# mirams/PyHillFit

Measured on NVIDIA B200. Metric: chain-iterations/sec (all chains, device-timed), higher is better.
Workload: dtype f64

## Files before the change

### pyhillfit_b200/csrc/phf_math.cuh

```cuda
#pragma once
#include <cstdint>
#include <cuda_runtime.h>
#include <math_constants.h>

#include "phf_fastmath.cuh"

#define PHF_DI __device__ __forceinline__
#if PHF_FM_TABLE_MODE == 1
#define PHF_STAGE_FASTMATH_TABLE(T)                                   \
    __shared__ __align__(16) double T##_smem[PHF_FM_TABLE_SIZE];      \
    phf::fm::stage_table(T##_smem);                                   \
    __syncthreads();                                                  \
    const double *const T = T##_smem
#elif PHF_FM_LUT
#define PHF_STAGE_FASTMATH_TABLE(T)                                                                     \
    __shared__ __align__(16) double T##_lut[PHF_FM_LUT_SIZE];                                           \
    for (int i_ = threadIdx.x; i_ < PHF_FM_LUT_SIZE; i_ += blockDim.x) T##_lut[i_] = phf::fm::kFmLut[i_]; \
    __syncthreads();                                                                                    \
    const double *const T = T##_lut
#else
#define PHF_STAGE_FASTMATH_TABLE(T) const double *const T = phf::fm::kFmTable
#endif

namespace phf {

constexpr double kSigmaLower = 1e-3;
constexpr double kPic50ExpRate = 0.2;
constexpr double kPic50ExpLower = -3.0;
constexpr double kHillLower = 0.0;
constexpr double kHillUpper = 10.0;
constexpr double kSigmaShapeM1 = 4.0;
constexpr double kSigmaScale = (6.0 - 1e-3) / (5.0 - 1.0);
constexpr double kLn10Hi = 2.302585092994045901e+00;
constexpr double kLn10Lo = -2.170756223382249351e-16;
constexpr double kSqrtHalf = 7.071067811865475244e-01;
constexpr double kPivotFloor = 1e-12;

__device__ __forceinline__ double guarded_pivot(double s, double diag)
{
    const double fl = kPivotFloor * diag;
    return s > fl ? s : fl;
}

PHF_DI double adapt_gamma(const double *T, uint32_t t, uint32_t adapt_when)
{
    return t > adapt_when ? fm::exp_clamped(T, -0.6 * fm::log_pos(T, (double)(t - adapt_when) + 1.0)) : 0.0;
}

template <int G>
PHF_DI unsigned group_mask()
{
    return G == 32 ? 0xffffffffu : (((1u << (G & 31)) - 1u) << (threadIdx.x & 31u & ~(unsigned)(G - 1)));
}

template <int G>
PHF_DI double group_sum(double v, unsigned mask)
{
#pragma unroll
    for (int o = G / 2; o > 0; o >>= 1) v += __shfl_xor_sync(mask, v, o, G);
    return v;
}

struct Philox4 {
    uint32_t w[4];
};

#ifndef PHF_PHILOX_ROUNDS
#define PHF_PHILOX_ROUNDS 10
#endif
PHF_DI Philox4 philox4x32_10(uint32_t c0, uint32_t c1, uint32_t c2, uint32_t c3, uint32_t k0, uint32_t k1)
{
#pragma unroll
    for (int r = 0; r < PHF_PHILOX_ROUNDS; ++r) {
        const uint32_t hi0 = __umulhi(0xD2511F53u, c0), lo0 = 0xD2511F53u * c0;
        const uint32_t hi1 = __umulhi(0xCD9E8D57u, c2), lo1 = 0xCD9E8D57u * c2;
        c0 = hi1 ^ c1 ^ k0;
        c1 = lo1;
        c2 = hi0 ^ c3 ^ k1;
        c3 = lo0;
        k0 += 0x9E3779B9u;
        k1 += 0xBB67AE85u;
    }
    Philox4 o;
    o.w[0] = c0; o.w[1] = c1; o.w[2] = c2; o.w[3] = c3;
    return o;
}

PHF_DI Philox4 philox_call(uint64_t seed, uint64_t chain, uint32_t t, uint32_t j)
{
    return philox4x32_10(t, j, (uint32_t)chain, (uint32_t)(chain >> 32), (uint32_t)seed, (uint32_t)(seed >> 32));
}

PHF_DI double uniform53(uint32_t w0, uint32_t w1)
{
    const unsigned long long v = (((unsigned long long)w0 << 32) | w1) >> 11;
    return fma((double)v, 0x1p-53, 0x1p-54);
}

PHF_DI void box_muller(const double *T, uint32_t a, uint32_t b, double &z0, double &z1)
{
    const double u1 = fma((double)a, 0x1p-32, 0x1p-32);
    const double r = fm::sqrt_nonneg(-2.0 * fm::log_pos(T, u1));
    double s, c;
    fm::sincos_turn32(T, b, s, c);
    z0 = r * c;
    z1 = r * s;
}

PHF_DI double log_ndtr_nonpos(const double *T, double z) { return fm::log_ndtr_nonpos(T, z); }

PHF_DI double ndtr(double a)
{
    const double x = a * kSqrtHalf, z = fabs(x);
    double y;
    if (z < 1.0)
        y = 0.5 + 0.5 * erf(x);
    else {
        y = 0.5 * erfc(z);
        if (x > 0) y = 1.0 - y;
    }
    return y;
}

PHF_DI void ln_ic50(double pic50, double &hi, double &lo)
{
    const double a = 6.0 - pic50;
    hi = a * kLn10Hi;
    lo = fma(a, kLn10Lo, fma(a, kLn10Hi, -hi));
}

template <bool ZERO_POW = true>
PHF_DI double hill_ratio_pow(const double *T, double lnc_hi, double lnc_lo, double lic_hi, double lic_lo, double hill)
{
    const double L = (lnc_hi - lic_hi) + (lnc_lo - lic_lo);
    const double x = fm::exp_clamped(T, hill * L);
    return (ZERO_POW && hill == 0.0) ? 1.0 : x;
}

PHF_DI double hill_response(double x) { return fma(-100.0, fm::rcp(1.0 + x), 100.0); }

}
```

### pyhillfit_b200/csrc/phf_single.cu

```cuda
#include "phf_common.cuh"
#include "phf_single.cuh"

namespace phf {

template <int MODEL>
__global__ void __launch_bounds__(128) log_target_batch_kernel(int64_t n, const double *__restrict__ theta,
                                                               const int32_t *__restrict__ dataset_id,
                                                               const double *__restrict__ temperature,
                                                               const phf_dataset *__restrict__ datasets,
                                                               const phf_dose_group *__restrict__ groups,
                                                               double *__restrict__ log_target,
                                                               double *__restrict__ loglik_t1)
{
    constexpr int D = SingleDims<MODEL>::D;
    PHF_STAGE_FASTMATH_TABLE(T);
    const int64_t i = (int64_t)blockIdx.x * blockDim.x + threadIdx.x;
    if (i >= n) return;
    double th[D];
#pragma unroll
    for (int k = 0; k < D; ++k) th[k] = theta[i * D + k];
    const phf_dataset ds = datasets[dataset_id[i]];
    double lt, l1;
    single_log_target<MODEL>(T, th, groups + ds.group_begin, ds.n_groups, ds.pi_bit, ds.n_other_total, temperature[i],
                             lt, l1);
    log_target[i] = lt;
    if (loglik_t1) loglik_t1[i] = l1;
}

template <int MODEL>
__global__ void __launch_bounds__(128) am_single_init_kernel(int64_t n, const double *__restrict__ theta0,
                                                             const double *__restrict__ cov0,
                                                             const int32_t *__restrict__ dataset_id,
                                                             const double *__restrict__ temperature,
                                                             const phf_dataset *__restrict__ datasets,
                                                             const phf_dose_group *__restrict__ groups,
                                                             double *__restrict__ state)
{
    constexpr int D = SingleDims<MODEL>::D, NT = SingleDims<MODEL>::NT, NF = SingleDims<MODEL>::NF;
    PHF_STAGE_FASTMATH_TABLE(T);
    const int64_t i = (int64_t)blockIdx.x * blockDim.x + threadIdx.x;
    if (i >= n) return;
    double th[D];
#pragma unroll
    for (int k = 0; k < D; ++k) th[k] = theta0[i * D + k];
    const phf_dataset ds = datasets[dataset_id[i]];
    double lt, l1;
    single_log_target<MODEL>(T, th, groups + ds.group_begin, ds.n_groups, ds.pi_bit, ds.n_other_total, temperature[i],
                             lt, l1);
    double *s = state + i * NF;
#pragma unroll
    for (int k = 0; k < D; ++k) {
        s[k] = th[k];
        s[PHF_STATE_MEAN(D) + k] = th[k];
    }
    s[PHF_STATE_LOG_TARGET(D)] = lt;
    s[PHF_STATE_LOGLIK_T1(D)] = l1;
    {
        int q = 0;
#pragma unroll
        for (int r = 0; r < D; ++r)
#pragma unroll
            for (int c2 = 0; c2 <= r; ++c2, ++q) {
                const double v = cov0[i * NT + q];
                s[PHF_STATE_COV(D) + q] = (r == c2 && !(v > 0.0) && v == v) ? PHF_COV0_DIAG_FLOOR : v;
            }
    }
    s[PHF_STATE_LOGA(D)] = 0.0;
    s[PHF_STATE_LOGLIK_T1_SUM(D)] = 0.0;
    s[PHF_STATE_N_ACCEPTED(D)] = 0.0;
}

struct ChainConst {
    const phf_dose_group *grp;
    int ng;
    double pi_bit, n_other_total, temp;
    uint32_t thinning, adapt_when, burn_rows, row_base;
    int reset_mean;
    PrepView pv;
    double *out;
    size_t row_stride;
    bool active;
};

template <int MODEL, int G>
PHF_DI void am_step(const double *T, const ChainConst &cc, ChainRegs<MODEL> &s, const Draws<SingleDims<MODEL>::D> &dr,
                    double gam, uint32_t t, int gl, unsigned mask, uint32_t &until_save, uint32_t &row)
{
    constexpr int D = SingleDims<MODEL>::D;
    double star[D];
    propose<MODEL>(T, s.th, s.cov, s.loga, dr.z, star);

    double lt_star, l1_star;
    single_log_target_lanes<MODEL, G, true, true>(T, star, cc.grp, cc.ng, cc.pi_bit, cc.n_other_total, cc.temp, gl, mask,
                                                  lt_star, l1_star, cc.pv);
    const bool accepted = dr.log_u < lt_star - s.lt;
    if (accepted) {
#pragma unroll
        for (int k = 0; k < D; ++k) s.th[k] = star[k];
        s.lt = lt_star;
        s.l1 = l1_star;
        s.n_acc += 1.0;
    }

    if (cc.reset_mean && t == cc.adapt_when) {
#pragma unroll
        for (int k = 0; k < D; ++k) s.mean[k] = s.th[k];
    }
    adapt_update<D>(s.mean, s.cov, s.loga, s.th, gam, (accepted ? 1.0 : 0.0) - 0.25);

    if (--until_save == 0u) {
        until_save = cc.thinning;
        ++row;
        if (cc.out && cc.active && row >= cc.row_base) {
            double *o = cc.out + (size_t)(row - cc.row_base) * cc.row_stride;
#pragma unroll
            for (int k = 0; k <= D; ++k)
                if ((k & (G - 1)) == gl) o[k] = k < D ? s.th[k < D ? k : 0] : s.lt;
        }
        if (row >= cc.burn_rows) s.l1_sum += s.l1;
    }
}

constexpr int kOrderClasses = 8;
constexpr int kOrderMaxGrid = 4096;

__device__ __forceinline__ int ordered_block_index(int cta_chains, const int32_t *__restrict__ dataset_id,
                                                   const phf_dataset *__restrict__ datasets,
                                                   const phf_dose_group *__restrict__ groups)
{
    __shared__ unsigned char cls[kOrderMaxGrid];
    __shared__ int count[kOrderClasses], my_class, my_rank, chosen;
    const int tid = threadIdx.x, n_ctas = gridDim.x;
    if (tid < kOrderClasses) count[tid] = 0;
    __syncthreads();
    for (int b = tid; b < n_ctas; b += blockDim.x) {
        const phf_dataset ds = datasets[dataset_id[(int64_t)b * cta_chains]];
        int w = ds.n_groups > 4 ? ds.n_groups - 4 : 0;
        for (int g = 0; g < ds.n_groups && g < 16; ++g) {
            const phf_dose_group &Gd = groups[ds.group_begin + g];
            w += (Gd.n0 > 0.0 ? 1 : 0) + (Gd.n100 > 0.0 ? 1 : 0);
        }
        w = w < kOrderClasses ? w : kOrderClasses - 1;
        cls[b] = (unsigned char)w;
        atomicAdd(&count[w], 1);
    }
    __syncthreads();
    if (tid == 0) {
        int p = blockIdx.x, c = kOrderClasses - 1;
        for (; c > 0 && p >= count[c]; --c) p -= count[c];
        my_class = c;
        my_rank = p;
    }
    __syncthreads();
    if (tid < 32) {
        const int want = my_class, rank = my_rank;
        int seen = 0;
        for (int base = 0; base < n_ctas; base += 32) {
            const int b = base + tid;
            const unsigned m = __ballot_sync(0xffffffffu, b < n_ctas && cls[b] == want);
            const int here = __popc(m);
            if (seen + here > rank) {
                if (tid == 0) chosen = base + (int)__fns(m, 0, rank - seen + 1);
                break;
            }
            seen += here;
        }
    }
    __syncthreads();
    return chosen;
}

template <int MODEL, int G, int MINB>
__global__ void __launch_bounds__(128, MINB)
    am_single_kernel(phf_am_config cfg, int64_t n, double *__restrict__ state, const int32_t *__restrict__ dataset_id,
                     const double *__restrict__ temperature, const phf_dataset *__restrict__ datasets,
                     const phf_dose_group *__restrict__ groups, double *__restrict__ samples, int ordered)
{
    constexpr int D = SingleDims<MODEL>::D, NF = SingleDims<MODEL>::NF;
    extern __shared__ __align__(16) unsigned char smem_raw[];
    phf_dose_group *sgroups = reinterpret_cast<phf_dose_group *>(smem_raw);
    PHF_STAGE_FASTMATH_TABLE(T);

    const int cta_chains = blockDim.x / G;
    const int64_t first = (int64_t)(ordered ? ordered_block_index(cta_chains, dataset_id, datasets, groups)
                                            : (int)blockIdx.x) * cta_chains;
    const int64_t chain = first + threadIdx.x / G;
    const int gl = threadIdx.x & (G - 1);
    const bool active = chain < n;
    const int64_t c = active ? chain : n - 1;
    const unsigned lane = threadIdx.x & 31u;
    const unsigned mask = 0xffffffffu;

    const phf_dataset ds = datasets[dataset_id[c]];
    ChainConst cc;
    cc.grp = ds.n_groups > 0 ? groups + ds.group_begin : groups;
    if (cfg.stage_groups > 0) {
        const int64_t last = min(first + (int64_t)cta_chains, n) - 1;
        const phf_dataset d_lo = datasets[dataset_id[first]];
        const phf_dataset d_hi = datasets[dataset_id[last]];
        const int g_lo = d_lo.group_begin, g_hi = d_hi.group_begin + d_hi.n_groups;
        const bool fits = (g_hi - g_lo) <= cfg.stage_groups && g_hi > g_lo && ds.group_begin >= g_lo &&
                          ds.group_begin + ds.n_groups <= g_hi;
        const int all_fit = __syncthreads_and(fits ? 1 : 0);
        if (all_fit) {
            const double2 *src = reinterpret_cast<const double2 *>(groups + g_lo);
            double2 *dst = reinterpret_cast<double2 *>(sgroups);
            const int nvec = (g_hi - g_lo) * 4;
            for (int v = threadIdx.x; v < nvec; v += blockDim.x) dst[v] = __ldg(src + v);
            __syncthreads();
            cc.grp = sgroups + (ds.n_groups > 0 ? ds.group_begin - g_lo : 0);
        }
    }
    cc.ng = ds.n_groups;
    cc.pi_bit = ds.pi_bit;
    cc.n_other_total = ds.n_other_total;
    cc.temp = temperature[c];
    cc.thinning = cfg.thinning;
    cc.adapt_when = cfg.adapt_when;
    cc.burn_rows = cfg.burn_rows;
    cc.reset_mean = cfg.reset_mean_at_adapt;
    cc.active = active;
    const uint64_t chain_id = cfg.chain_id_base + (uint64_t)c;

    double *sp = state + c * NF;
    ChainRegs<MODEL> s;
    s.load(sp);

    uint32_t t = cfg.t0;
    uint32_t until_save = cfg.thinning - (t % cfg.thinning);
    uint32_t row = t / cfg.thinning;
    cc.row_base = first_row_written(cfg);
    const bool row_major = cfg.sample_layout == PHF_SAMPLES_ROW_MAJOR;
    cc.out = samples ? samples + (row_major ? (size_t)c : (size_t)c * cfg.rows_capacity) * (D + 1) : nullptr;
    cc.row_stride = row_major ? (size_t)n * (D + 1) : (size_t)(D + 1);

    double *const slots = reinterpret_cast<double *>(smem_raw + (size_t)cfg.stage_groups * sizeof(phf_dose_group));
    double *const gam_base = slots + (G > 1 ? (size_t)blockDim.x * (D + 1) : 0);
    double *const gam_slots = gam_base + (size_t)(threadIdx.x & ~31u);
    {
        constexpr int U = 4 / G;
        double2 *const prep = reinterpret_cast<double2 *>(gam_base + blockDim.x) + threadIdx.x;
        bool both = false;
#pragma unroll
        for (int u = 0; u < U; ++u)
            prepare_group<MODEL>(cc.grp, gl + u * G, cc.ng, prep + (size_t)(u * kPrepPairs) * blockDim.x, (int)blockDim.x, both);
        cc.pv = PrepView{prep, (int)blockDim.x, both};
    }

    double *const my_slot = slots + (size_t)threadIdx.x * (D + 1);
    const double *const chain_slots = slots + (size_t)(threadIdx.x & ~(unsigned)(G - 1)) * (D + 1);
    for (uint32_t it = 0; it < cfg.n_iters; ++it) {
        ++t;
        if ((it & 31u) == 0u) {
            const double gam_lane = adapt_gamma(T, t + lane, cfg.adapt_when);
            __syncwarp();
            gam_slots[lane] = gam_lane;
            __syncwarp();
        }
        const double gam = gam_slots[it & 31u];
        Draws<D> dr;
        if (G == 1) {
            dr = make_draws<D>(T, cfg.seed, chain_id, t);
        } else {
            const int slot = (int)(it & (uint32_t)(G - 1));
            if (slot == 0) {
                const Draws<D> mine = make_draws<D>(T, cfg.seed, chain_id, t + (uint32_t)gl);
                __syncwarp();
                my_slot[0] = mine.log_u;
#pragma unroll
                for (int k = 0; k < D; ++k) my_slot[1 + k] = mine.z[k];
                __syncwarp();
            }
            const double *src = chain_slots + slot * (D + 1);
            dr.log_u = src[0];
#pragma unroll
            for (int k = 0; k < D; ++k) dr.z[k] = src[1 + k];
        }
        am_step<MODEL, G>(T, cc, s, dr, gam, t, gl, mask, until_save, row);
    }

    if (active && gl == 0) s.store(sp);
}

template <int MODEL, int G, int MINB>
static int launch_am_single(const phf_am_config &cfg, int64_t n, int block, double *state, const int32_t *dataset_id,
                            const double *temperature, const phf_dataset *datasets, const phf_dose_group *groups,
                            double *samples, cudaStream_t s)
{
    constexpr int D = SingleDims<MODEL>::D;
    auto kern = am_single_kernel<MODEL, G, MINB>;
    const size_t smem = (size_t)cfg.stage_groups * sizeof(phf_dose_group) +
                        (G > 1 ? (size_t)block * (D + 1) * sizeof(double) : 0) + (size_t)block * sizeof(double) +
                        (size_t)block * (4 / G) * 64;
    if (int rc = allow_dynamic_smem(kern, smem)) return rc;
    const int cta_chains = block / G;
    const unsigned grid = (unsigned)((n + cta_chains - 1) / cta_chains);
    const int ordered = cfg.cta_order == 0 && grid > (unsigned)sm_count() && grid <= (unsigned)kOrderMaxGrid;
    kern<<<grid, block, smem, s>>>(cfg, n, state, dataset_id, temperature, datasets, groups, samples, ordered);
    count_launch();
    return check_launch("am_single_kernel");
}

int am_single_spec_launch(const phf_am_config &cfg, int lanes, int depth, int64_t n, int block, double *state,
                          const int32_t *dataset_id, const double *temperature, const phf_dataset *datasets,
                          const phf_dose_group *groups, double *samples, cudaStream_t s);

}

using namespace phf;

extern "C" int phf_log_target_batch(int model, int64_t n, const double *theta, const int32_t *dataset_id,
                                    const double *temperature, const phf_dataset *datasets,
                                    const phf_dose_group *groups, double *log_target, double *loglik_t1, void *stream)
{
    if (model != 1 && model != 2) return set_error(PHF_EINVAL, "model must be 1 or 2");
    if (n < 0 || (n > 0 && (!theta || !dataset_id || !temperature || !datasets || !groups || !log_target)))
        return set_error(PHF_EINVAL, "phf_log_target_batch: null pointer");
    if (n == 0) return PHF_OK;
    const int block = 128;
    const unsigned grid = (unsigned)((n + block - 1) / block);
    cudaStream_t s = (cudaStream_t)stream;
    if (model == 1)
        log_target_batch_kernel<1><<<grid, block, 0, s>>>(n, theta, dataset_id, temperature, datasets, groups,
                                                          log_target, loglik_t1);
    else
        log_target_batch_kernel<2><<<grid, block, 0, s>>>(n, theta, dataset_id, temperature, datasets, groups,
                                                          log_target, loglik_t1);
    count_launch();
    return check_launch("log_target_batch_kernel");
}

extern "C" int phf_am_single_init(int model, int64_t n_chains, const double *theta0, const double *cov0_tri,
                                  const int32_t *dataset_id, const double *temperature, const phf_dataset *datasets,
                                  const phf_dose_group *groups, double *state, void *stream)
{
    if (model != 1 && model != 2) return set_error(PHF_EINVAL, "model must be 1 or 2");
    if (n_chains < 0 || (n_chains > 0 && (!theta0 || !cov0_tri || !dataset_id || !temperature || !datasets ||
                                          !groups || !state)))
        return set_error(PHF_EINVAL, "phf_am_single_init: null pointer");
    if (n_chains == 0) return PHF_OK;
    const int block = 128;
    const unsigned grid = (unsigned)((n_chains + block - 1) / block);
    cudaStream_t s = (cudaStream_t)stream;
    if (model == 1)
        am_single_init_kernel<1><<<grid, block, 0, s>>>(n_chains, theta0, cov0_tri, dataset_id, temperature,
                                                        datasets, groups, state);
    else
        am_single_init_kernel<2><<<grid, block, 0, s>>>(n_chains, theta0, cov0_tri, dataset_id, temperature,
                                                        datasets, groups, state);
    count_launch();
    return check_launch("am_single_init_kernel");
}

extern "C" int phf_am_single_lanes(int64_t n_chains)
{
    const int64_t sms = sm_count();
    if (n_chains * 4 <= sms * 128) return 4;
    if (n_chains * 2 <= sms * 384) return 2;
    return 1;
}

extern "C" int phf_am_single_speculation(int64_t n_chains, int lanes)
{
    const int64_t sms = sm_count();
    if (lanes < 1) lanes = 1;
    if (lanes * 4 <= 32 && n_chains * lanes * 4 <= sms * 256) return 4;
    if (lanes * 2 <= 32 && n_chains * lanes * 2 <= sms * 256) return 2;
    return 1;
}

extern "C" int phf_am_single_shape(int64_t n_chains, int32_t lanes, int32_t speculation, int32_t *lanes_out,
                                   int32_t *speculation_out)
{
    if (!lanes_out || !speculation_out) return set_error(PHF_EINVAL, "phf_am_single_shape: null output");
    if (lanes != 0 && lanes != 1 && lanes != 2 && lanes != 4)
        return set_error(PHF_EINVAL, "cfg.lanes_per_chain must be 0 (auto), 1, 2 or 4");
    if (speculation != 0 && speculation != 1 && speculation != 2 && speculation != 4 && speculation != 8)
        return set_error(PHF_EINVAL, "cfg.speculation must be 0 (auto), 1 (none), 2, 4 or 8");
    if (lanes == 0 && speculation == 0) {
        lanes = phf_am_single_lanes(n_chains);
        if (lanes == 4) lanes = 2;
        speculation = phf_am_single_speculation(n_chains, lanes);
    } else if (lanes == 0) {
        lanes = phf_am_single_lanes(n_chains);
    } else if (speculation == 0) {
        speculation = phf_am_single_speculation(n_chains, lanes);
    }
    if (lanes * speculation > 32 || (speculation == 8 && lanes == 1))
        return set_error(PHF_EINVAL, "lanes_per_chain x speculation: 1, 2, 4 lanes x depth 2, 4 (8 with 2 or 4 lanes)");
    *lanes_out = lanes;
    *speculation_out = speculation;
    return PHF_OK;
}

extern "C" int phf_am_single_run(const phf_am_config *cfg, int64_t n_chains, double *state,
                                 const int32_t *dataset_id, const double *temperature, const phf_dataset *datasets,
                                 const phf_dose_group *groups, double *samples, void *stream)
{
    if (!cfg) return set_error(PHF_EINVAL, "phf_am_single_run: cfg is NULL");
    if (cfg->model != 1 && cfg->model != 2) return set_error(PHF_EINVAL, "cfg.model must be 1 or 2");
    if (int rc = check_run_config(*cfg, samples != nullptr)) return rc;
    if (n_chains < 0 || (n_chains > 0 && (!state || !dataset_id || !temperature || !datasets || !groups)))
        return set_error(PHF_EINVAL, "phf_am_single_run: null pointer");
    if (n_chains == 0 || cfg->n_iters == 0) return PHF_OK;

    int32_t lanes = 0, depth = 0;
    if (int rc = phf_am_single_shape(n_chains, cfg->lanes_per_chain, cfg->speculation, &lanes, &depth)) return rc;
    int block = cfg->block_threads;
    if (block <= 0) block = depth > 1 ? 128 : default_block_threads(n_chains * lanes);
    if (block % 32 != 0 || block > 128)
        return set_error(PHF_EINVAL, "cfg.block_threads must be a multiple of 32, at most 128");
    if (cfg->stage_groups < 0) return set_error(PHF_EINVAL, "cfg.stage_groups must be >= 0");
    if (depth > 1 && (uint64_t)cfg->t0 + cfg->n_iters > 0xFFFFFF00ull)
        return set_error(PHF_EINVAL, "iteration counter overflow (speculative form)");
    if (depth > 1)
        return am_single_spec_launch(*cfg, lanes, depth, n_chains, block, state, dataset_id, temperature, datasets, groups,
                                     samples, (cudaStream_t)stream);
    cudaStream_t s = (cudaStream_t)stream;
    const int minb = cfg->min_ctas_hint > 0 ? cfg->min_ctas_hint : 3;
#define PHF_AM_CASE(M, G, MINB)                                                                                  \
    if (cfg->model == M && lanes == G && minb == MINB)                                                                       \
        return launch_am_single<M, G, MINB>(*cfg, n_chains, block, state, dataset_id, temperature, datasets, groups, \
                                            samples, s)
    PHF_AM_CASE(1, 1, 3);
    PHF_AM_CASE(1, 2, 3);
    PHF_AM_CASE(1, 4, 3);
    PHF_AM_CASE(2, 1, 3);
    PHF_AM_CASE(2, 2, 3);
    PHF_AM_CASE(2, 4, 3);
    PHF_AM_CASE(1, 1, 2);
    PHF_AM_CASE(1, 2, 2);
    PHF_AM_CASE(1, 4, 2);
    PHF_AM_CASE(2, 1, 2);
    PHF_AM_CASE(2, 2, 2);
    PHF_AM_CASE(2, 4, 2);
    PHF_AM_CASE(1, 1, 4);
    PHF_AM_CASE(1, 2, 4);
    PHF_AM_CASE(1, 4, 4);
    PHF_AM_CASE(2, 1, 4);
    PHF_AM_CASE(2, 2, 4);
    PHF_AM_CASE(2, 4, 4);
    PHF_AM_CASE(2, 4, 6);
#undef PHF_AM_CASE
    return set_error(PHF_EINVAL, "no kernel variant for this (model, lanes, occupancy hint)");
}

extern "C" int phf_am_single_resident_ctas(int model, int lanes, int block_threads, int64_t smem_bytes)
{
    int n = 0;
    cudaError_t e = cudaErrorInvalidValue;
#define PHF_OCC_CASE(M, G)                                                                                           \
    if (model == M && lanes == G)                                                                                    \
        e = cudaOccupancyMaxActiveBlocksPerMultiprocessor(&n, am_single_kernel<M, G, 3>, block_threads, (size_t)smem_bytes)
    PHF_OCC_CASE(1, 1);
    PHF_OCC_CASE(1, 2);
    PHF_OCC_CASE(1, 4);
    PHF_OCC_CASE(2, 1);
    PHF_OCC_CASE(2, 2);
    PHF_OCC_CASE(2, 4);
#undef PHF_OCC_CASE
    if (e) return set_cuda_error(e, "phf_am_single_resident_ctas");
    return n;
}
```

### pyhillfit_b200/csrc/phf_single.cuh

```cuda
#pragma once
#include "../../include/pyhillfit_b200.h"
#include "phf_common.cuh"
#include "phf_math.cuh"

namespace phf {

template <int MODEL>
struct SingleDims {
    static constexpr int D = MODEL == 1 ? 2 : 3;
    static constexpr int NT = D * (D + 1) / 2;
    static constexpr int NF = PHF_STATE_SIZE(D);
};

template <int MODEL, bool PW = false>
PHF_DI void dose_group_terms(const double *T, const phf_dose_group &Gd, double hill, double lic_hi, double lic_lo, double inv_ic50,
                             double inv_s, double &e2, double &cens)
{
    const double x = MODEL == 2 ? hill_ratio_pow(T, Gd.lnc_hi, Gd.lnc_lo, lic_hi, lic_lo, hill) : Gd.conc * inv_ic50;
    const double p = hill_response(x);
    const double r = Gd.ybar - p;
    e2 += fma(Gd.n_other * r, r, Gd.ss);
    const bool has0 = Gd.n0 > 0.0, has100 = Gd.n100 > 0.0;
    if (has0 || has100) {
        const double z = has0 ? (0.0 - p) * inv_s : (p - 100.0) * inv_s;
        cens = fma(has0 ? Gd.n0 : Gd.n100, PW ? fm::log_ndtr_nonpos_pw(T, z) : fm::log_ndtr_nonpos(T, z), cens);
        if (has0 && has100) {
            const double z2 = (p - 100.0) * inv_s;
            cens = fma(Gd.n100, PW ? fm::log_ndtr_nonpos_pw(T, z2) : fm::log_ndtr_nonpos(T, z2), cens);
        }
    }
}

template <bool VOTE, bool PW = false>
PHF_DI double censored_pair(const double *T, double z0, double w0, double z1, double w1)
{
    auto lphi = [&](double z) { return PW ? fm::log_ndtr_nonpos_pw(T, z) : fm::log_ndtr_nonpos(T, z); };
    const bool c0 = w0 > 0.0, c1 = w1 > 0.0;
    bool two = c0 && c1, one = c0 || c1;
    if (VOTE) {
        two = __any_sync(0xffffffffu, two) != 0;
        one = __any_sync(0xffffffffu, one) != 0;
    }
    double acc = 0.0;
    if (two) {
        acc = fma(w1, lphi(z1), w0 * lphi(z0));
    } else if (one) {
        acc = (c0 ? w0 : w1) * lphi(c0 ? z0 : z1);
    }
    return acc;
}

constexpr int kPrepPairs = 4;

template <int MODEL>
PHF_DI void prepare_group(const phf_dose_group *__restrict__ grp, int g, int ng, double2 *dst, int stride, bool &both)
{
    double a0 = 0.0, a1 = 0.0, ybar = 0.0, n_other = 0.0, ss = 0.0, csign = 1.0, coff = -100.0, cw = 0.0;
    if (g < ng) {
        const phf_dose_group Gd = grp[g];
        a0 = MODEL == 2 ? Gd.lnc_hi : Gd.conc;
        a1 = Gd.lnc_lo;
        ybar = Gd.ybar;
        n_other = Gd.n_other;
        ss = Gd.ss;
        const bool has0 = Gd.n0 > 0.0, has100 = Gd.n100 > 0.0;
        csign = has0 ? -1.0 : 1.0;
        coff = has0 ? 0.0 : -100.0;
        cw = has0 ? Gd.n0 : (has100 ? Gd.n100 : 0.0);
        both = both || (has0 && has100);
    }
    dst[0 * stride] = make_double2(a0, a1);
    dst[1 * stride] = make_double2(ybar, n_other);
    dst[2 * stride] = make_double2(ss, csign);
    dst[3 * stride] = make_double2(coff, cw);
}

struct PrepView {
    const double2 *rec;
    int stride;
    bool both_kinds;
};

template <int MODEL, int G, bool VOTE, bool PREP = false>
PHF_DI void single_log_target_lanes(const double *T, const double *th, const phf_dose_group *__restrict__ grp, int ng,
                                    double pi_bit, double n_other_total, double temperature, int gl, unsigned mask,
                                    double &log_target, double &loglik_t1, const PrepView pv = PrepView{nullptr, 0, false})
{
    const double pic50 = th[0];
    const double hill = MODEL == 2 ? th[1] : 1.0;
    const double sigma = th[MODEL == 2 ? 2 : 1];
    const bool sigma_ok = sigma > kSigmaLower;
    const double sg = sigma_ok ? sigma : 1.0;
    const double inv_s = fm::rcp(sg);
    const double sm = sg - kSigmaLower;
    double log_s = 0.0, log_sm = 0.0, lane_log = 0.0;
    if (G >= 2) {
        lane_log = fm::log_pos(T, gl == 0 ? sg : sm);
    } else {
        log_s = fm::log_pos(T, sg);
        log_sm = fm::log_pos(T, sm);
    }
    bool in_support = sigma_ok && (pic50 >= kPic50ExpLower);
    if (MODEL == 2) in_support = in_support && (hill >= kHillLower) && (hill <= kHillUpper);

    double lic_hi = 0.0, lic_lo = 0.0, inv_ic50 = 0.0;
    if (MODEL == 2)
        ln_ic50(pic50, lic_hi, lic_lo);
    else
        inv_ic50 = fm::exp10_clamped(T, pic50 - 6.0);

    constexpr int U = 4 / G;
    constexpr bool PW = VOTE && G >= 2;
    double e2 = 0.0, cens = 0.0;
    double zc[U], wc[U], pu[U];
    bool both_kinds = false;
#pragma unroll
    for (int u = 0; u < U; ++u) {
        if (PREP) {
            const double2 r0 = pv.rec[(u * kPrepPairs + 0) * pv.stride], r1 = pv.rec[(u * kPrepPairs + 1) * pv.stride];
            const double2 r2 = pv.rec[(u * kPrepPairs + 2) * pv.stride], r3 = pv.rec[(u * kPrepPairs + 3) * pv.stride];
            const double x = MODEL == 2 ? hill_ratio_pow<!VOTE>(T, r0.x, r0.y, lic_hi, lic_lo, hill) : r0.x * inv_ic50;
            const double p = hill_response(x);
            const double r = r1.x - p;
            e2 += fma(r1.y * r, r, r2.x);
            zc[u] = fma(r2.y, p, r3.x) * inv_s;
            wc[u] = r3.y;
            pu[u] = p;
            continue;
        }
        const int g = gl + u * G;
        const bool on = g < ng;
        const phf_dose_group *Gp = grp + (on ? g : 0);
        const double x = MODEL == 2 ? hill_ratio_pow<!VOTE>(T, Gp->lnc_hi, Gp->lnc_lo, lic_hi, lic_lo, hill)
                                    : Gp->conc * inv_ic50;
        const double p = hill_response(x);
        const double r = Gp->ybar - p;
        const double gauss = fma(Gp->n_other * r, r, Gp->ss);
        e2 += on ? gauss : 0.0;
        const double n0 = Gp->n0, n100 = Gp->n100;
        const bool has0 = on && n0 > 0.0, has100 = on && n100 > 0.0;
        zc[u] = (has0 ? 0.0 - p : p - 100.0) * inv_s;
        wc[u] = has0 ? n0 : (has100 ? n100 : 0.0);
        pu[u] = p;
        both_kinds = both_kinds || (has0 && has100);
    }
    if (U == 1) {
        cens = censored_pair<VOTE, PW>(T, zc[0], wc[0], zc[0], 0.0);
    } else {
#pragma unroll
        for (int u = 0; u + 1 < U; u += 2) cens += censored_pair<VOTE, PW>(T, zc[u], wc[u], zc[u + 1], wc[u + 1]);
    }
    if (PREP ? pv.both_kinds : both_kinds) {
#pragma unroll
        for (int u = 0; u < U; ++u) {
            const int g = gl + u * G;
            if (g < ng && grp[g].n0 > 0.0 && grp[g].n100 > 0.0)
                cens = fma(grp[g].n100, PW ? fm::log_ndtr_nonpos_pw(T, (pu[u] - 100.0) * inv_s)
                                           : fm::log_ndtr_nonpos(T, (pu[u] - 100.0) * inv_s), cens);
        }
    }
    for (int g = gl + U * G; g < ng; g += G) {
        const phf_dose_group Gd = grp[g];
        dose_group_terms<MODEL, PW>(T, Gd, hill, lic_hi, lic_lo, inv_ic50, inv_s, e2, cens);
    }
    double raw, log_sm4;
    if (G >= 2) {
        double lik = fma(-e2, 0.5 * inv_s * inv_s, cens);
        lik = gl == 0 ? fma(-n_other_total, lane_log, lik - pi_bit) : lik;
        double pri = gl == 1 ? kSigmaShapeM1 * lane_log : 0.0;
        raw = group_sum<G>(lik, mask);
        log_sm4 = group_sum<G>(pri, mask);
    } else {
        raw = fma(-e2, 0.5 * inv_s * inv_s, fma(-n_other_total, log_s, cens - pi_bit));
        log_sm4 = kSigmaShapeM1 * log_sm;
    }
    const double prior = fma(-kPic50ExpRate, pic50, fma(-sm, 1.0 / kSigmaScale, log_sm4));
    loglik_t1 = sigma_ok ? raw : -CUDART_INF;
    const double post = temperature == 0.0 ? prior : fma(temperature, raw, prior);
    log_target = in_support ? post : -CUDART_INF;
}

template <int MODEL>
PHF_DI void single_log_target(const double *T, const double *th, const phf_dose_group *__restrict__ grp, int ng,
                              double pi_bit, double n_other_total, double temperature, double &log_target,
                              double &loglik_t1)
{
    single_log_target_lanes<MODEL, 1, false>(T, th, grp, ng, pi_bit, n_other_total, temperature, 0, 0xffffffffu,
                                             log_target, loglik_t1);
}


template <int D>
struct Draws {
    double log_u;
    double z[D];
};

template <int D>
PHF_DI Draws<D> make_draws(const double *T, uint64_t seed, uint64_t chain_id, uint32_t t)
{
    Draws<D> dr;
    const Philox4 r0 = philox_call(seed, chain_id, t, 0u);
    dr.log_u = fm::log_pos(T, uniform53(r0.w[0], r0.w[1]));
    box_muller(T, r0.w[2], r0.w[3], dr.z[0], dr.z[1]);
    if (D == 3) {
        const Philox4 r1 = philox_call(seed, chain_id, t, 1u);
        double unused;
        box_muller(T, r1.w[0], r1.w[1], dr.z[D - 1], unused);
    }
    return dr;
}

template <int MODEL>
struct ChainRegs {
    static constexpr int D = SingleDims<MODEL>::D, NT = SingleDims<MODEL>::NT;
    double th[D], mean[D], cov[NT];
    double lt, l1, loga, l1_sum, n_acc;

    PHF_DI void load(const double *sp)
    {
#pragma unroll
        for (int k = 0; k < D; ++k) {
            th[k] = sp[k];
            mean[k] = sp[PHF_STATE_MEAN(D) + k];
        }
        lt = sp[PHF_STATE_LOG_TARGET(D)];
        l1 = sp[PHF_STATE_LOGLIK_T1(D)];
#pragma unroll
        for (int k = 0; k < NT; ++k) cov[k] = sp[PHF_STATE_COV(D) + k];
        loga = sp[PHF_STATE_LOGA(D)];
        l1_sum = sp[PHF_STATE_LOGLIK_T1_SUM(D)];
        n_acc = sp[PHF_STATE_N_ACCEPTED(D)];
    }
    PHF_DI void store(double *sp) const
    {
#pragma unroll
        for (int k = 0; k < D; ++k) {
            sp[k] = th[k];
            sp[PHF_STATE_MEAN(D) + k] = mean[k];
        }
        sp[PHF_STATE_LOG_TARGET(D)] = lt;
        sp[PHF_STATE_LOGLIK_T1(D)] = l1;
#pragma unroll
        for (int k = 0; k < NT; ++k) sp[PHF_STATE_COV(D) + k] = cov[k];
        sp[PHF_STATE_LOGA(D)] = loga;
        sp[PHF_STATE_LOGLIK_T1_SUM(D)] = l1_sum;
        sp[PHF_STATE_N_ACCEPTED(D)] = n_acc;
    }
};

template <int D>
PHF_DI void adapt_update(double *mean, double *cov, double &loga, const double *th, double gam, double acc_minus_quarter)
{
    const double omg = 1.0 - gam;
    double dv[D];
#pragma unroll
    for (int k = 0; k < D; ++k) dv[k] = th[k] - mean[k];
    int q = 0;
#pragma unroll
    for (int i = 0; i < D; ++i)
#pragma unroll
        for (int j = 0; j <= i; ++j, ++q) cov[q] = fma(gam, dv[i] * dv[j], omg * cov[q]);
#pragma unroll
    for (int k = 0; k < D; ++k) mean[k] = fma(gam, th[k], omg * mean[k]);
    loga = fma(gam, acc_minus_quarter, loga);
}

template <typename Kernel>
static int allow_dynamic_smem(Kernel kern, size_t smem)
{
    if (smem > 200 * 1024) return set_error(PHF_EINVAL, "cfg.stage_groups needs more than 200 KB of shared memory");
    cudaError_t e;
    if (smem > 40 * 1024 && (e = cudaFuncSetAttribute(kern, cudaFuncAttributeMaxDynamicSharedMemorySize, (int)smem)))
        return set_cuda_error(e, "cudaFuncSetAttribute");
    return PHF_OK;
}

template <int MODEL>
PHF_DI void propose(const double *T, const double *th, const double *cov, double loga, const double *z, double *star)
{
    constexpr int D = SingleDims<MODEL>::D;
    const double sc = fm::exp_clamped(T, 0.5 * loga);
    const double r0 = fm::rsqrt(cov[0]);
    const double l00 = cov[0] * r0, l10 = cov[1] * r0;
    const double s11 = guarded_pivot(fma(-l10, l10, cov[2]), cov[2]);
    const double r1 = fm::rsqrt(s11);
    const double l11 = s11 * r1;
    star[0] = fma(sc, l00 * z[0], th[0]);
    star[1] = fma(sc, fma(l10, z[0], l11 * z[1]), th[1]);
    if (D == 3) {
        const double l20 = cov[3] * r0;
        const double l21 = fma(-l20, l10, cov[4]) * r1;
        const double s22 = guarded_pivot(fma(-l21, l21, fma(-l20, l20, cov[5])), cov[5]);
        const double l22 = s22 * fm::rsqrt(s22);
        star[D - 1] = fma(sc, fma(l20, z[0], fma(l21, z[1], l22 * z[D - 1])), th[D - 1]);
    }
}

}
```

### pyhillfit_b200/csrc/phf_single_spec.cu

```cuda
#include "phf_common.cuh"
#include "phf_single.cuh"

namespace phf {

template <int MODEL, int E, int S>
__global__ void __launch_bounds__(128, 3)
    am_single_spec_kernel(phf_am_config cfg, int64_t n, double *__restrict__ state,
                          const int32_t *__restrict__ dataset_id, const double *__restrict__ temperature,
                          const phf_dataset *__restrict__ datasets, const phf_dose_group *__restrict__ groups,
                          double *__restrict__ samples)
{
    constexpr int D = SingleDims<MODEL>::D, NT = SingleDims<MODEL>::NT, NF = SingleDims<MODEL>::NF;
    constexpr int G = E * S;
    constexpr int R = 2 * G;
    constexpr int W = D + 2;
    static_assert(G <= 32 && (G & (G - 1)) == 0, "E x S lanes per chain, a power of two, at most a warp");
    extern __shared__ __align__(16) unsigned char smem_raw[];
    phf_dose_group *sgroups = reinterpret_cast<phf_dose_group *>(smem_raw);
    PHF_STAGE_FASTMATH_TABLE(T);

    const int cta_chains = blockDim.x / G;
    const int64_t first = (int64_t)blockIdx.x * cta_chains;
    const int64_t chain = first + threadIdx.x / G;
    const int gl = threadIdx.x & (G - 1);
    const int g = gl / E;
    const int el = gl & (E - 1);
    const bool active = chain < n;
    const int64_t c = active ? chain : n - 1;
    const unsigned lane = threadIdx.x & 31u;
    const unsigned cbase = lane & ~(unsigned)(G - 1);
    constexpr unsigned full = 0xffffffffu;

    const phf_dataset ds = datasets[dataset_id[c]];
    const phf_dose_group *grp = ds.n_groups > 0 ? groups + ds.group_begin : groups;
    if (cfg.stage_groups > 0) {
        const int64_t last = min(first + (int64_t)cta_chains, n) - 1;
        const phf_dataset d_lo = datasets[dataset_id[first]];
        const phf_dataset d_hi = datasets[dataset_id[last]];
        const int g_lo = d_lo.group_begin, g_hi = d_hi.group_begin + d_hi.n_groups;
        const bool fits = (g_hi - g_lo) <= cfg.stage_groups && g_hi > g_lo && ds.group_begin >= g_lo &&
                          ds.group_begin + ds.n_groups <= g_hi;
        const int all_fit = __syncthreads_and(fits ? 1 : 0);
        if (all_fit) {
            const double2 *src = reinterpret_cast<const double2 *>(groups + g_lo);
            double2 *dst = reinterpret_cast<double2 *>(sgroups);
            const int nvec = (g_hi - g_lo) * 4;
            for (int v = threadIdx.x; v < nvec; v += blockDim.x) dst[v] = __ldg(src + v);
            __syncthreads();
            grp = sgroups + (ds.n_groups > 0 ? ds.group_begin - g_lo : 0);
        }
    }
    const int ng = ds.n_groups;
    const double pi_bit = ds.pi_bit, n_other_total = ds.n_other_total, temp = temperature[c];
    const uint64_t chain_id = cfg.chain_id_base + (uint64_t)c;

    double *sp = state + c * NF;
    ChainRegs<MODEL> s;
    s.load(sp);

    uint32_t t = cfg.t0;
    const uint32_t t_end = cfg.t0 + cfg.n_iters;
    RowCursor rows(cfg, c, n, D, samples);

    double *const ring = reinterpret_cast<double *>(smem_raw + (size_t)cfg.stage_groups * sizeof(phf_dose_group)) +
                         (size_t)(threadIdx.x / G) * (R * W);
    uint32_t filled = t;
    PrepView pv;
    {
        constexpr int U = 4 / E;
        double2 *const prep = reinterpret_cast<double2 *>(
                                  reinterpret_cast<double *>(smem_raw + (size_t)cfg.stage_groups * sizeof(phf_dose_group)) +
                                  (size_t)cta_chains * (R * W)) + threadIdx.x;
        bool both = false;
#pragma unroll
        for (int u = 0; u < U; ++u)
            prepare_group<MODEL>(grp, el + u * E, ng, prep + (size_t)(u * kPrepPairs) * blockDim.x, (int)blockDim.x, both);
        pv = PrepView{prep, (int)blockDim.x, both};
    }

    for (;;) {
        const bool alive = t < t_end;
        if (!__any_sync(full, alive)) break;

        if (__any_sync(full, alive && (filled - t) < (uint32_t)S)) {
            __syncwarp();
            if ((filled - t) <= (uint32_t)(R - G)) {
                const uint32_t ti = filled + 1u + (uint32_t)gl;
                const Draws<D> mine = make_draws<D>(T, cfg.seed, chain_id, ti);
                const double gam = adapt_gamma(T, ti, cfg.adapt_when);
                double *e = ring + (ti % (uint32_t)R) * W;
                e[0] = mine.log_u;
#pragma unroll
                for (int k = 0; k < D; ++k) e[1 + k] = mine.z[k];
                e[1 + D] = gam;
                filled += (uint32_t)G;
            }
            __syncwarp();
        }

        double gam[S];
#pragma unroll
        for (int j = 0; j < S; ++j) gam[j] = ring[((t + 1u + (uint32_t)j) % (uint32_t)R) * W + 1 + D];
        const uint32_t ti = t + 1u + (uint32_t)g;
        double log_u, z[D];
        {
            const double *e = ring + (ti % (uint32_t)R) * W;
            log_u = e[0];
#pragma unroll
            for (int k = 0; k < D; ++k) z[k] = e[1 + k];
        }

        double h_mean[D], h_cov[NT], h_loga = s.loga;
#pragma unroll
        for (int k = 0; k < D; ++k) h_mean[k] = s.mean[k];
#pragma unroll
        for (int k = 0; k < NT; ++k) h_cov[k] = s.cov[k];
#pragma unroll
        for (int j = 0; j + 1 < S; ++j) {
            const bool mine = j < g;
            if (mine && cfg.reset_mean_at_adapt && (t + 1u + (uint32_t)j) == cfg.adapt_when) {
#pragma unroll
                for (int k = 0; k < D; ++k) h_mean[k] = s.th[k];
            }
            adapt_update<D>(h_mean, h_cov, h_loga, s.th, mine ? gam[j] : 0.0, -0.25);
        }

        double star[D];
        propose<MODEL>(T, s.th, h_cov, h_loga, z, star);
        double lt_star, l1_star;
        single_log_target_lanes<MODEL, E, true, true>(T, star, grp, ng, pi_bit, n_other_total, temp, el, full, lt_star,
                                                      l1_star, pv);

        const uint32_t left = alive ? t_end - t : 0u;
        const int n_valid = left < (uint32_t)S ? (int)left : S;
        const bool acc = g < n_valid && (log_u < lt_star - s.lt);
        const unsigned votes = (__ballot_sync(full, acc) >> cbase) & (G == 32 ? 0xffffffffu : ((1u << (G & 31)) - 1u));
        const bool fin_acc = votes != 0u;
        const int f = fin_acc ? (__ffs((int)votes) - 1) / E : 0;
        const int k_adv = fin_acc ? f + 1 : n_valid;
        const int last_g = k_adv > 0 ? k_adv - 1 : 0;

        uint32_t j_save = rows.until_save;
        while (j_save < (uint32_t)k_adv) {
            ++rows.row;
            if (double *o = rows.dest(active))
                for (int k = gl; k <= D; k += G) o[k] = k == 0 ? s.th[0] : (k == 1 ? s.th[1] : (k < D ? s.th[D - 1] : s.lt));
            if (rows.row >= cfg.burn_rows) s.l1_sum += s.l1;
            j_save += cfg.thinning;
        }

        {
            const int src_h = (int)cbase + last_g * E;
#pragma unroll
            for (int k = 0; k < D; ++k) s.mean[k] = __shfl_sync(full, h_mean[k], src_h);
#pragma unroll
            for (int k = 0; k < NT; ++k) s.cov[k] = __shfl_sync(full, h_cov[k], src_h);
            s.loga = __shfl_sync(full, h_loga, src_h);
            {
                const int src = fin_acc ? (int)cbase + f * E : (int)lane;
#pragma unroll
                for (int k = 0; k < D; ++k) {
                    const double v = __shfl_sync(full, star[k], src);
                    s.th[k] = fin_acc ? v : s.th[k];
                }
                const double v_lt = __shfl_sync(full, lt_star, src), v_l1 = __shfl_sync(full, l1_star, src);
                s.lt = fin_acc ? v_lt : s.lt;
                s.l1 = fin_acc ? v_l1 : s.l1;
                s.n_acc += fin_acc ? 1.0 : 0.0;
            }
            const uint32_t t_last = t + (uint32_t)k_adv;
            if (k_adv > 0 && cfg.reset_mean_at_adapt && t_last == cfg.adapt_when) {
#pragma unroll
                for (int k = 0; k < D; ++k) s.mean[k] = s.th[k];
            }
            const double gam_last = k_adv > 0 ? ring[(t_last % (uint32_t)R) * W + 1 + D] : 0.0;
            adapt_update<D>(s.mean, s.cov, s.loga, s.th, gam_last, (fin_acc ? 1.0 : 0.0) - 0.25);
        }
        if (k_adv > 0 && j_save == (uint32_t)k_adv) {
            ++rows.row;
            if (double *o = rows.dest(active))
                for (int k = gl; k <= D; k += G) o[k] = k == 0 ? s.th[0] : (k == 1 ? s.th[1] : (k < D ? s.th[D - 1] : s.lt));
            if (rows.row >= cfg.burn_rows) s.l1_sum += s.l1;
            j_save += cfg.thinning;
        }
        rows.until_save = j_save - (uint32_t)k_adv;
        t += (uint32_t)k_adv;
    }

    if (active && gl == 0) s.store(sp);
}

template <int MODEL, int E, int S>
static int launch_spec(const phf_am_config &cfg, int64_t n, int block, double *state, const int32_t *dataset_id,
                       const double *temperature, const phf_dataset *datasets, const phf_dose_group *groups,
                       double *samples, cudaStream_t s)
{
    constexpr int D = SingleDims<MODEL>::D, G = E * S;
    auto kern = am_single_spec_kernel<MODEL, E, S>;
    const int cta_chains = block / G;
    const size_t smem = (size_t)cfg.stage_groups * sizeof(phf_dose_group) +
                        (size_t)cta_chains * (2 * G) * (D + 2) * sizeof(double) + (size_t)block * (4 / E) * 64;
    if (int rc = allow_dynamic_smem(kern, smem)) return rc;
    const unsigned grid = (unsigned)((n + cta_chains - 1) / cta_chains);
    kern<<<grid, block, smem, s>>>(cfg, n, state, dataset_id, temperature, datasets, groups, samples);
    count_launch();
    return check_launch("am_single_spec_kernel");
}

int am_single_spec_launch(const phf_am_config &cfg, int lanes, int depth, int64_t n, int block, double *state,
                          const int32_t *dataset_id, const double *temperature, const phf_dataset *datasets,
                          const phf_dose_group *groups, double *samples, cudaStream_t s)
{
#define PHF_SPEC_CASE(M, E, S)                                                                                       \
    if (cfg.model == M && lanes == E && depth == S)                                                                  \
        return launch_spec<M, E, S>(cfg, n, block, state, dataset_id, temperature, datasets, groups, samples, s)
    PHF_SPEC_CASE(1, 1, 2); PHF_SPEC_CASE(2, 1, 2);
    PHF_SPEC_CASE(1, 1, 4); PHF_SPEC_CASE(2, 1, 4);
    PHF_SPEC_CASE(1, 2, 2); PHF_SPEC_CASE(2, 2, 2);
    PHF_SPEC_CASE(1, 2, 4); PHF_SPEC_CASE(2, 2, 4);
    PHF_SPEC_CASE(1, 2, 8); PHF_SPEC_CASE(2, 2, 8);
    PHF_SPEC_CASE(1, 4, 2); PHF_SPEC_CASE(2, 4, 2);
    PHF_SPEC_CASE(1, 4, 4); PHF_SPEC_CASE(2, 4, 4);
    PHF_SPEC_CASE(1, 4, 8); PHF_SPEC_CASE(2, 4, 8);
#undef PHF_SPEC_CASE
    return set_error(PHF_EINVAL, "no speculative kernel for this (model, lanes_per_chain, speculation): lanes 1, 2, 4 x "
                                 "depth 2, 4 (and 8 with 2 or 4 lanes)");
}

}
```

Baseline: 17.21 billion.

## Factor per-chain Philox rounds and precompute round keys on host

Precomputes the Philox round keys once on the host and passes them as a grid-constant kernel parameter. It also factors the parts of the first rounds that depend only on the chain id and call index into per-chain values computed once. Each per-iteration draw then shares the rounds that depend only on t across both Philox calls. The aim is fewer integer multiplies per iteration in the RNG-heavy MCMC loop, while keeping the output bit-identical. The cost is more live registers for the cached per-chain values and keys, which could hurt occupancy.

```diff
diff --git a/pyhillfit_b200/csrc/phf_math.cuh b/pyhillfit_b200/csrc/phf_math.cuh
--- a/pyhillfit_b200/csrc/phf_math.cuh
+++ b/pyhillfit_b200/csrc/phf_math.cuh
@@ -4,6 +4,7 @@
 #include <math_constants.h>
 
 #include "phf_fastmath.cuh"
+#include "phf_philox.cuh"
 
 #define PHF_DI __device__ __forceinline__
 #if PHF_FM_TABLE_MODE == 1
@@ -61,36 +62,6 @@
     return v;
 }
 
-struct Philox4 {
-    uint32_t w[4];
-};
-
-#ifndef PHF_PHILOX_ROUNDS
-#define PHF_PHILOX_ROUNDS 10
-#endif
-PHF_DI Philox4 philox4x32_10(uint32_t c0, uint32_t c1, uint32_t c2, uint32_t c3, uint32_t k0, uint32_t k1)
-{
-#pragma unroll
-    for (int r = 0; r < PHF_PHILOX_ROUNDS; ++r) {
-        const uint32_t hi0 = __umulhi(0xD2511F53u, c0), lo0 = 0xD2511F53u * c0;
-        const uint32_t hi1 = __umulhi(0xCD9E8D57u, c2), lo1 = 0xCD9E8D57u * c2;
-        c0 = hi1 ^ c1 ^ k0;
-        c1 = lo1;
-        c2 = hi0 ^ c3 ^ k1;
-        c3 = lo0;
-        k0 += 0x9E3779B9u;
-        k1 += 0xBB67AE85u;
-    }
-    Philox4 o;
-    o.w[0] = c0; o.w[1] = c1; o.w[2] = c2; o.w[3] = c3;
-    return o;
-}
-
-PHF_DI Philox4 philox_call(uint64_t seed, uint64_t chain, uint32_t t, uint32_t j)
-{
-    return philox4x32_10(t, j, (uint32_t)chain, (uint32_t)(chain >> 32), (uint32_t)seed, (uint32_t)(seed >> 32));
-}
-
 PHF_DI double uniform53(uint32_t w0, uint32_t w1)
 {
     const unsigned long long v = (((unsigned long long)w0 << 32) | w1) >> 11;
diff --git a/pyhillfit_b200/csrc/phf_philox.cuh b/pyhillfit_b200/csrc/phf_philox.cuh
--- /dev/null
+++ b/pyhillfit_b200/csrc/phf_philox.cuh
@@ -0,0 +1,140 @@
+#pragma once
+#include <cstdint>
+
+#if defined(__CUDACC__)
+#define PHF_PHILOX_FN __host__ __device__ __forceinline__
+#else
+#define PHF_PHILOX_FN static inline
+#endif
+
+#ifndef PHF_PHILOX_ROUNDS
+#define PHF_PHILOX_ROUNDS 10
+#endif
+
+namespace phf {
+
+struct Philox4 {
+    uint32_t w[4];
+};
+
+constexpr uint32_t kPhiloxM0 = 0xD2511F53u;
+constexpr uint32_t kPhiloxM1 = 0xCD9E8D57u;
+constexpr uint32_t kPhiloxW0 = 0x9E3779B9u;
+constexpr uint32_t kPhiloxW1 = 0xBB67AE85u;
+
+PHF_PHILOX_FN void philox_mul(uint32_t m, uint32_t c, uint32_t &hi, uint32_t &lo)
+{
+    const uint64_t p = (uint64_t)m * c;
+    hi = (uint32_t)(p >> 32);
+    lo = (uint32_t)p;
+}
+
+PHF_PHILOX_FN uint32_t philox_mulhi(uint32_t m, uint32_t c)
+{
+#if defined(__CUDA_ARCH__)
+    return __umulhi(m, c);
+#else
+    return (uint32_t)(((uint64_t)m * c) >> 32);
+#endif
+}
+
+PHF_PHILOX_FN Philox4 philox4x32_10(uint32_t c0, uint32_t c1, uint32_t c2, uint32_t c3, uint32_t k0, uint32_t k1)
+{
+#if defined(__CUDA_ARCH__)
+#pragma unroll
+#endif
+    for (int r = 0; r < PHF_PHILOX_ROUNDS; ++r) {
+        const uint32_t hi0 = philox_mulhi(kPhiloxM0, c0), lo0 = kPhiloxM0 * c0;
+        const uint32_t hi1 = philox_mulhi(kPhiloxM1, c2), lo1 = kPhiloxM1 * c2;
+        c0 = hi1 ^ c1 ^ k0;
+        c1 = lo1;
+        c2 = hi0 ^ c3 ^ k1;
+        c3 = lo0;
+        k0 += kPhiloxW0;
+        k1 += kPhiloxW1;
+    }
+    Philox4 o;
+    o.w[0] = c0; o.w[1] = c1; o.w[2] = c2; o.w[3] = c3;
+    return o;
+}
+
+PHF_PHILOX_FN Philox4 philox_call(uint64_t seed, uint64_t chain, uint32_t t, uint32_t j)
+{
+    return philox4x32_10(t, j, (uint32_t)chain, (uint32_t)(chain >> 32), (uint32_t)seed, (uint32_t)(seed >> 32));
+}
+
+struct PhiloxKeys {
+    uint32_t k0[PHF_PHILOX_ROUNDS], k1[PHF_PHILOX_ROUNDS];
+};
+
+PHF_PHILOX_FN PhiloxKeys philox_keys(uint64_t seed)
+{
+    PhiloxKeys K;
+    uint32_t k0 = (uint32_t)seed, k1 = (uint32_t)(seed >> 32);
+    for (int r = 0; r < PHF_PHILOX_ROUNDS; ++r, k0 += kPhiloxW0, k1 += kPhiloxW1) {
+        K.k0[r] = k0;
+        K.k1[r] = k1;
+    }
+    return K;
+}
+
+template <int NCALLS>
+struct PhiloxChain {
+    uint32_t x1;
+    uint32_t x0;
+    uint32_t y[NCALLS];
+    uint32_t z[NCALLS];
+};
+
+template <int NCALLS>
+PHF_PHILOX_FN PhiloxChain<NCALLS> philox_chain(const PhiloxKeys &K, uint64_t chain)
+{
+    PhiloxChain<NCALLS> C;
+    uint32_t hi, lo;
+    philox_mul(kPhiloxM1, (uint32_t)chain, hi, lo);
+    C.x1 = (uint32_t)(chain >> 32) ^ K.k1[0];
+    C.x0 = lo ^ K.k0[1];
+    for (int j = 0; j < NCALLS; ++j) {
+        uint32_t phi, plo;
+        philox_mul(kPhiloxM0, hi ^ (uint32_t)j ^ K.k0[0], phi, plo);
+        C.y[j] = phi ^ K.k1[1];
+        C.z[j] = plo;
+    }
+    return C;
+}
+
+template <int NCALLS>
+PHF_PHILOX_FN void philox_calls(const PhiloxKeys &K, const PhiloxChain<NCALLS> &C, uint32_t t, Philox4 *out)
+{
+    static_assert(PHF_PHILOX_ROUNDS >= 3, "the factored form shares rounds 0 to 2");
+    uint32_t h, l;
+    philox_mul(kPhiloxM0, t, h, l);
+    const uint32_t r0c2 = h ^ C.x1, r0c3 = l;
+    philox_mul(kPhiloxM1, r0c2, h, l);
+    const uint32_t r1c0 = h ^ C.x0, r1c1 = l;
+    uint32_t s_hi, s_lo;
+    philox_mul(kPhiloxM0, r1c0, s_hi, s_lo);
+#if defined(__CUDA_ARCH__)
+#pragma unroll
+#endif
+    for (int j = 0; j < NCALLS; ++j) {
+        const uint32_t r1c2 = r0c3 ^ C.y[j];
+        philox_mul(kPhiloxM1, r1c2, h, l);
+        uint32_t c0 = h ^ r1c1 ^ K.k0[2], c1 = l, c2 = s_hi ^ C.z[j] ^ K.k1[2], c3 = s_lo;
+#if defined(__CUDA_ARCH__)
+#pragma unroll
+#endif
+        for (int r = 3; r < PHF_PHILOX_ROUNDS; ++r) {
+            uint32_t hi0, lo0, hi1, lo1;
+            philox_mul(kPhiloxM0, c0, hi0, lo0);
+            philox_mul(kPhiloxM1, c2, hi1, lo1);
+            c0 = hi1 ^ c1 ^ K.k0[r];
+            c1 = lo1;
+            c2 = hi0 ^ c3 ^ K.k1[r];
+            c3 = lo0;
+        }
+        out[j].w[0] = c0; out[j].w[1] = c1; out[j].w[2] = c2; out[j].w[3] = c3;
+    }
+}
+
+}
diff --git a/pyhillfit_b200/csrc/phf_single.cu b/pyhillfit_b200/csrc/phf_single.cu
--- a/pyhillfit_b200/csrc/phf_single.cu
+++ b/pyhillfit_b200/csrc/phf_single.cu
@@ -174,7 +174,8 @@
 __global__ void __launch_bounds__(128, MINB)
     am_single_kernel(phf_am_config cfg, int64_t n, double *__restrict__ state, const int32_t *__restrict__ dataset_id,
                      const double *__restrict__ temperature, const phf_dataset *__restrict__ datasets,
-                     const phf_dose_group *__restrict__ groups, double *__restrict__ samples, int ordered)
+                     const phf_dose_group *__restrict__ groups, double *__restrict__ samples, int ordered,
+                     const __grid_constant__ PhiloxKeys keys)
 {
     constexpr int D = SingleDims<MODEL>::D, NF = SingleDims<MODEL>::NF;
     extern __shared__ __align__(16) unsigned char smem_raw[];
@@ -220,7 +221,7 @@
     cc.burn_rows = cfg.burn_rows;
     cc.reset_mean = cfg.reset_mean_at_adapt;
     cc.active = active;
-    const uint64_t chain_id = cfg.chain_id_base + (uint64_t)c;
+    const DrawChain<D> pc = philox_chain<D == 3 ? 2 : 1>(keys, cfg.chain_id_base + (uint64_t)c);
 
     double *sp = state + c * NF;
     ChainRegs<MODEL> s;
@@ -260,11 +261,11 @@
         const double gam = gam_slots[it & 31u];
         Draws<D> dr;
         if (G == 1) {
-            dr = make_draws<D>(T, cfg.seed, chain_id, t);
+            dr = make_draws<D>(T, keys, pc, t);
         } else {
             const int slot = (int)(it & (uint32_t)(G - 1));
             if (slot == 0) {
-                const Draws<D> mine = make_draws<D>(T, cfg.seed, chain_id, t + (uint32_t)gl);
+                const Draws<D> mine = make_draws<D>(T, keys, pc, t + (uint32_t)gl);
                 __syncwarp();
                 my_slot[0] = mine.log_u;
 #pragma unroll
@@ -296,7 +297,8 @@
     const int cta_chains = block / G;
     const unsigned grid = (unsigned)((n + cta_chains - 1) / cta_chains);
     const int ordered = cfg.cta_order == 0 && grid > (unsigned)sm_count() && grid <= (unsigned)kOrderMaxGrid;
-    kern<<<grid, block, smem, s>>>(cfg, n, state, dataset_id, temperature, datasets, groups, samples, ordered);
+    kern<<<grid, block, smem, s>>>(cfg, n, state, dataset_id, temperature, datasets, groups, samples, ordered,
+                                   philox_keys(cfg.seed));
     count_launch();
     return check_launch("am_single_kernel");
 }
diff --git a/pyhillfit_b200/csrc/phf_single.cuh b/pyhillfit_b200/csrc/phf_single.cuh
--- a/pyhillfit_b200/csrc/phf_single.cuh
+++ b/pyhillfit_b200/csrc/phf_single.cuh
@@ -197,16 +197,19 @@
 };
 
 template <int D>
-PHF_DI Draws<D> make_draws(const double *T, uint64_t seed, uint64_t chain_id, uint32_t t)
+using DrawChain = PhiloxChain<D == 3 ? 2 : 1>;
+
+template <int D>
+PHF_DI Draws<D> make_draws(const double *T, const PhiloxKeys &K, const DrawChain<D> &pc, uint32_t t)
 {
     Draws<D> dr;
-    const Philox4 r0 = philox_call(seed, chain_id, t, 0u);
-    dr.log_u = fm::log_pos(T, uniform53(r0.w[0], r0.w[1]));
-    box_muller(T, r0.w[2], r0.w[3], dr.z[0], dr.z[1]);
-    if (D == 3) {
-        const Philox4 r1 = philox_call(seed, chain_id, t, 1u);
+    Philox4 r[D == 3 ? 2 : 1];
+    philox_calls(K, pc, t, r);
+    dr.log_u = fm::log_pos(T, uniform53(r[0].w[0], r[0].w[1]));
+    box_muller(T, r[0].w[2], r[0].w[3], dr.z[0], dr.z[1]);
+    if constexpr (D == 3) {
         double unused;
-        box_muller(T, r1.w[0], r1.w[1], dr.z[D - 1], unused);
+        box_muller(T, r[1].w[0], r[1].w[1], dr.z[D - 1], unused);
     }
     return dr;
 }
diff --git a/pyhillfit_b200/csrc/phf_single_spec.cu b/pyhillfit_b200/csrc/phf_single_spec.cu
--- a/pyhillfit_b200/csrc/phf_single_spec.cu
+++ b/pyhillfit_b200/csrc/phf_single_spec.cu
@@ -8,7 +8,7 @@
     am_single_spec_kernel(phf_am_config cfg, int64_t n, double *__restrict__ state,
                           const int32_t *__restrict__ dataset_id, const double *__restrict__ temperature,
                           const phf_dataset *__restrict__ datasets, const phf_dose_group *__restrict__ groups,
-                          double *__restrict__ samples)
+                          double *__restrict__ samples, const __grid_constant__ PhiloxKeys keys)
 {
     constexpr int D = SingleDims<MODEL>::D, NT = SingleDims<MODEL>::NT, NF = SingleDims<MODEL>::NF;
     constexpr int G = E * S;
@@ -52,7 +52,7 @@
     }
     const int ng = ds.n_groups;
     const double pi_bit = ds.pi_bit, n_other_total = ds.n_other_total, temp = temperature[c];
-    const uint64_t chain_id = cfg.chain_id_base + (uint64_t)c;
+    const DrawChain<D> pc = philox_chain<D == 3 ? 2 : 1>(keys, cfg.chain_id_base + (uint64_t)c);
 
     double *sp = state + c * NF;
     ChainRegs<MODEL> s;
@@ -86,7 +86,7 @@
             __syncwarp();
             if ((filled - t) <= (uint32_t)(R - G)) {
                 const uint32_t ti = filled + 1u + (uint32_t)gl;
-                const Draws<D> mine = make_draws<D>(T, cfg.seed, chain_id, ti);
+                const Draws<D> mine = make_draws<D>(T, keys, pc, ti);
                 const double gam = adapt_gamma(T, ti, cfg.adapt_when);
                 double *e = ring + (ti % (uint32_t)R) * W;
                 e[0] = mine.log_u;
@@ -202,7 +202,7 @@
                         (size_t)cta_chains * (2 * G) * (D + 2) * sizeof(double) + (size_t)block * (4 / E) * 64;
     if (int rc = allow_dynamic_smem(kern, smem)) return rc;
     const unsigned grid = (unsigned)((n + cta_chains - 1) / cta_chains);
-    kern<<<grid, block, smem, s>>>(cfg, n, state, dataset_id, temperature, datasets, groups, samples);
+    kern<<<grid, block, smem, s>>>(cfg, n, state, dataset_id, temperature, datasets, groups, samples, philox_keys(cfg.seed));
     count_launch();
     return check_launch("am_single_spec_kernel");
 }
```

Result: no change. 17.17 billion (median of 6 runs) (-0.2%).
